# axiom-crypto/halo2-lib

Hardware: AMD Instinct MI355X
Metric: create_proof constraints/sec (k=19 ECDSA configuration, halo2-ecc/configs/secp256k1/bench_ecdsa.config:1); MSM G1-adds/sec in `msm_2_20` (higher is better)
Workload: dtype u32 (254-bit Montgomery integers as 8x32 / 9x29-bit limbs); 1 GPU; BASELINE configs[3]: h2hip_plonk_create_proof, k=19 secp256k1-ECDSA shape (bench_ecdsa.config:1: 1 advice + 1 lookup + 1 constants column, lookup_bits 18), synthetic circuit-like witness resident in HBM; 1 step = 1 proof, bytes back on the host; constraints_per_proof=524280, msm_count=12, msm_size=524288, extended_k=21, degree=5, proof_bytes=960

## Files before the change

### halo2-lib_amd/csrc/internal.h

```cpp
#pragma once
#include <hip/hip_runtime.h>
#include <stdint.h>
#include <stdio.h>
#include <string.h>
#include <functional>
#include <map>
#include <string>
#include <vector>

#include "../../include/h2hip.h"
#include "ec.cuh"
#include "ec29.cuh"

namespace h2 {

void set_error(const char *fmt, ...);

#define H2_HIPCHK(expr)                                                                              \
    do {                                                                                             \
        hipError_t e__ = (expr);                                                                     \
        if (e__ != hipSuccess) {                                                                     \
            h2::set_error("%s:%d: %s -> %s", __FILE__, __LINE__, #expr, hipGetErrorString(e__));     \
            return H2HIP_ERR_HIP;                                                                    \
        }                                                                                            \
    } while (0)

#define H2_CHK(expr)                      \
    do {                                  \
        int r__ = (expr);                 \
        if (r__ != H2HIP_OK) return r__;  \
    } while (0)

#define H2_REQUIRE(cond, msg)                                        \
    do {                                                             \
        if (!(cond)) {                                               \
            h2::set_error("%s: invalid argument: %s", __func__, msg); \
            return H2HIP_ERR_INVALID;                                \
        }                                                            \
    } while (0)

struct DevBuf {
    void *p = nullptr;
    size_t cap = 0;
};

struct TwiddleSet {
    uint32_t log_n = 0, lo_bits = 0;
    Fr omega;
    void *t1 = nullptr;
    void *t2 = nullptr;
    void *direct[4] = {nullptr, nullptr, nullptr, nullptr};
    uint32_t direct_log_s[4] = {0, 0, 0, 0};
};

struct KernelStat {
    double total_ms = 0;
    uint64_t launches = 0;
    std::vector<std::pair<float, float>> spans;
};

}

struct h2hip_ctx {
    int device = 0;
    hipStream_t stream = nullptr;
    bool own_stream = false;
    int num_cus = 256;
    enum { WS_NTT = 0, WS_DIGITS, WS_COUNTS, WS_OFFSETS, WS_CURSOR, WS_SKEY, WS_SVAL, WS_BUCKETS, WS_PKEY0, WS_PVAL0, WS_PKEY1,
           WS_PVAL1, WS_SEG, WS_WIN, WS_OUT, WS_SCAN, WS_TMP0, WS_TMP1, WS_TMP2, WS_STAGE, WS_POSEIDON, WS_FBTABLE, WS_BATCH, WS_LK0, WS_LK1, WS_LK2, WS_LK3, WS_LK4, WS_LK5, WS_VANISH, WS_BATCH_BUCKETS, WS_COUNT };
    h2::DevBuf ws[WS_COUNT];
    std::vector<h2::TwiddleSet> twiddles;
    int msm_window_bits = 0;
    int msm_chunk = 0;
    int msm_seg = 4;
    int ntt_tile_bits = 10;
    int ntt_min_col_bits = 2;
    int ntt_full_table = 1;
    int ntt_tile_kernel = 1;
    int ntt_debug_skip = 0;
    int msm_quad_tails = 1;
    int msm_sort_threads = 1024;
    int msm_scatter_split = 0;
    int msm_scatter_full_lds = 0;
    bool is_lane = false;
    int msm_chunk_lone = -1;
    int msm_hist_split = 0;
    int msm_sort_groups = 0;
    int msm_hist_packed = 1;
    uint32_t pos_t = 0, pos_rf = 0, pos_rp = 0;
    bool profiling = false;
    std::string prof_filter;
    std::map<std::string, h2::KernelStat> stats;
    struct PendingLaunch {
        std::string name;
        hipEvent_t begin, end;
        bool ended;
    };
    std::vector<PendingLaunch> pending;
    std::vector<hipEvent_t> event_pool;
    hipEvent_t prof_ref = nullptr;
    bool own_prof_ref = false;
    h2hip_ctx *lane[4] = {nullptr, nullptr, nullptr, nullptr};
    hipEvent_t lane_ev[4] = {nullptr, nullptr, nullptr, nullptr};
    char *job_ring = nullptr;
    size_t job_ring_off = 0;
    std::function<int()> msm_mid_hook;
    size_t msm_mid_after = 0;
    std::function<int(size_t)> msm_col_hook;
    hipEvent_t fork_ev3 = nullptr;
    int plonk_lazy_upload = 1;
    hipEvent_t fork_ev2 = nullptr;
    std::function<int(hipEvent_t ev)> msm_tail_hook;
    hipEvent_t tail_ev = nullptr;
    int msm_lanes = 0;
    int plonk_tail_overlap = 1;
    int quotient_29 = 1;
    int plonk_permute_in_commit = 1;
    int clean_on_lane = 1;
    int kate_29 = 1;
    int kate_coeffs_per_lane = 0;
    int plonk_merge_products = 1;
    int plonk_shard_side = 1;
    int plonk_route_rows = 1;
    int plonk_early_intt = 1;
    int plonk_gate_before_join = 0;
    int msm_stagger_sorts = -1;
    hipEvent_t sorted_ev = nullptr;
    bool sorted_arm = false;
    int plonk_side_on_lanes = 1;
#ifdef H2_HIPEMU
    int plonk_warm_keygen = 0;
#else
    int plonk_warm_keygen = 1;
#endif
    int fr_invert_run = 0;
    int lookup_big_tile_bits = 19;
    int msm_quad_seg_max = 32768;
    int msm_defer_reduce = 1;
    int msm_fuse_cols = 0;
    hipStream_t clean_stream = nullptr;
    hipEvent_t clean_ev = nullptr, clean_ev1 = nullptr, used_ev = nullptr;
    void *clean_ptr[2] = {nullptr, nullptr};
    size_t clean_bytes[2] = {0, 0};
    hipEvent_t fork_ev = nullptr;
    hipEvent_t timer_ev[2] = {nullptr, nullptr};
    int msm_table_split = 1;
    int host_poll = 1;
    char *poll_host = nullptr;
    char *poll_dev = nullptr;
    unsigned long long poll_seq = 0;
    bool msm_lds_attr_set = false, lookup_lds_attr_set = false, ntt_lds_attr_set = false;
};

namespace h2 {
inline bool knob_pow2(int v) { return v > 0 && (v & (v - 1)) == 0; }
}
#define H2_INHERITED true
#define H2_PARENT_ONLY(why) false
#define H2_KNOB_TABLE(K)                                                                                                                          \
    K(msm_window_bits, H2_INHERITED, v == 0 || (v >= 4 && v <= 16), "0 (auto) or 4..16")                                                         \
    K(msm_chunk, H2_INHERITED, v == 0 || (v >= 2 && v <= 4096), "0 (auto) or 2..4096")                                                          \
    K(msm_chunk_lone, H2_INHERITED, v >= -1 && v <= 4096, "-1 (auto), 0 (the batch rule) or 1..4096")                                          \
    K(msm_seg, H2_INHERITED, h2::knob_pow2(v) && v <= 1024, "a power of two <= 1024")                                                          \
    K(msm_quad_tails, H2_INHERITED, v == 0 || v == 1, "0 or 1")                                                                                 \
    K(msm_quad_seg_max, H2_INHERITED, v >= 0, ">= 0")                                                                                           \
    K(msm_sort_threads, H2_INHERITED, v == 256 || v == 512 || v == 1024, "256, 512 or 1024")                                                   \
    K(msm_sort_groups, H2_INHERITED, v >= 0 && v <= 1024, "0 (auto) or 1..1024")                                                               \
    K(msm_hist_split, H2_INHERITED, v == 0 || (h2::knob_pow2(v) && v <= 64), "0 or a power of two <= 64")                                      \
    K(msm_hist_packed, H2_INHERITED, v == 0 || v == 1, "0 or 1")                                                                                \
    K(msm_scatter_split, H2_INHERITED, v == 0 || (h2::knob_pow2(v) && v <= 64), "0 (auto) or a power of two <= 64")                            \
    K(msm_scatter_full_lds, H2_INHERITED, v == 0 || v == 1, "0 or 1")                                                                           \
    K(msm_table_split, H2_INHERITED, v == 0 || v == 1, "0 or 1")                                                                                \
    K(msm_lanes, H2_PARENT_ONLY("read only by the batch driver, on the caller's context"), v >= 0 && v <= 4, "0 (auto) or 1..4")              \
    K(msm_stagger_sorts, H2_PARENT_ONLY("read only by the batch driver, on the caller's context"), v >= -1 && v <= 1, "-1 (auto), 0 or 1")     \
    K(msm_fuse_cols, H2_PARENT_ONLY("read only by the batch driver, on the caller's context"), v >= 0 && v <= (int)h2::MSM_MAX_COLS,           \
      "0 (auto) or 1..32")                                                                                                                        \
    K(msm_defer_reduce, H2_PARENT_ONLY("read only by the batch driver, on the caller's context"), v == 0 || v == 1, "0 or 1")                  \
    K(clean_on_lane, H2_PARENT_ONLY("read only by the batch driver, on the caller's context"), v == 0 || v == 1, "0 or 1")                     \
    K(ntt_tile_bits, H2_INHERITED, v >= 4 && v <= 10, "4..10")                                                                                  \
    K(ntt_min_col_bits, H2_INHERITED, v >= 0 && v <= 5, "0..5")                                                                                 \
    K(ntt_full_table, H2_INHERITED, v == 0 || v == 1, "0 or 1")                                                                                 \
    K(ntt_tile_kernel, H2_INHERITED, v == 0 || v == 1, "0 or 1")                                                                                \
    K(ntt_debug_skip, H2_INHERITED, v >= 0 && v <= 2, "0, 1 or 2")                                                                              \
    K(quotient_29, H2_INHERITED, v == 0 || v == 1, "0 or 1")                                                                                    \
    K(kate_29, H2_INHERITED, v == 0 || v == 1, "0 or 1")                                                                                        \
    K(kate_coeffs_per_lane, H2_INHERITED, v == 0 || v == 1 || v == 2 || v == 4 || v == 8, "0 (by length), 1, 2, 4 or 8")                       \
    K(fr_invert_run, H2_INHERITED, v >= 0 && v <= 1024, "0 (auto) or 1..1024")                                                                 \
    K(lookup_big_tile_bits, H2_INHERITED, v >= 12 && v <= 28, "12..28")                                                                         \
    K(host_poll, H2_INHERITED, v == 0 || v == 1, "0 or 1")                                                                                      \
    K(plonk_warm_keygen, H2_PARENT_ONLY("read only by h2hip_plonk_keygen"), v == 0 || v == 1, "0 or 1")                                       \
    K(plonk_tail_overlap, H2_PARENT_ONLY("read only by create_proof, on the caller's context"), v == 0 || v == 1, "0 or 1")                    \
    K(plonk_side_on_lanes, H2_PARENT_ONLY("read only by create_proof, on the caller's context"), v == 0 || v == 1, "0 or 1")                   \
    K(plonk_permute_in_commit, H2_PARENT_ONLY("read only by create_proof, on the caller's context"), v == 0 || v == 1, "0 or 1")               \
    K(plonk_merge_products, H2_PARENT_ONLY("read only by create_proof, on the caller's context"), v == 0 || v == 1, "0 or 1")                  \
    K(plonk_shard_side, H2_PARENT_ONLY("read only by create_proof, on the caller's context"), v >= 0 && v <= 2, "0, 1 or 2 (forced)")          \
    K(plonk_route_rows, H2_PARENT_ONLY("read only by create_proof, on the caller's context"), v == 0 || v == 1, "0 or 1")                      \
    K(plonk_lazy_upload, H2_PARENT_ONLY("read only by create_proof, on the caller's context"), v == 0 || v == 1, "0 or 1")                     \
    K(plonk_early_intt, H2_PARENT_ONLY("read only by create_proof, on the caller's context"), v == 0 || v == 1, "0 or 1")                      \
    K(plonk_gate_before_join, H2_PARENT_ONLY("read only by create_proof, on the caller's context"), v == 0 || v == 1, "0 or 1")

namespace h2 {
inline void inherit_knobs(h2hip_ctx *c, const h2hip_ctx *p) {
#define H2_KNOB_INHERIT(name, inherit, legal, domain) \
    if (inherit) c->name = p->name;
    H2_KNOB_TABLE(H2_KNOB_INHERIT)
#undef H2_KNOB_INHERIT
    c->profiling = p->profiling;
    c->prof_filter = p->prof_filter;
    c->prof_ref = p->prof_ref;
}
struct DeviceGuard {
    int prev = -1;
    bool switched = false;
    explicit DeviceGuard(const h2hip_ctx *c) {
        if (c && hipGetDevice(&prev) == hipSuccess && prev != c->device) switched = hipSetDevice(c->device) == hipSuccess;
    }
    ~DeviceGuard() {
        if (switched) hipSetDevice(prev);
    }
    DeviceGuard(const DeviceGuard &) = delete;
    DeviceGuard &operator=(const DeviceGuard &) = delete;
};
}
#define H2_DEVICE_GUARD(ctx) h2::DeviceGuard device_guard__(ctx)

struct h2hip_bases {
    h2::G1Affine *pts = nullptr;
    h2::G1Affine *pts29 = nullptr;
    bool split = false;
    size_t n = 0;
    uint32_t window_bits = 0;
    uint32_t tables = 1;
};

namespace h2 {
struct alignas(128) TableEntry29 {
    uint32_t x[9], y[9];
    uint32_t pad[14];
};
static_assert(sizeof(TableEntry29) == 128, "one entry per 128-byte line");
int ws_reserve(h2hip_ctx *ctx, int slot, size_t bytes, void **out);

void prof_begin(h2hip_ctx *ctx, const char *name);
void prof_end(h2hip_ctx *ctx);
bool prof_launch_events(h2hip_ctx *ctx, const char *name, hipEvent_t *start, hipEvent_t *stop);

int ntt_run(h2hip_ctx *ctx, Fr *a, uint32_t log_n, const Fr &omega, const Fr *in_override, uint64_t in_len, const Fr *in_scale3,
            const Fr *out_scale3);
int ntt_run_batch(h2hip_ctx *ctx, Fr *const *a, const Fr *const *in_override, size_t ncols, uint32_t log_n, const Fr &omega, uint64_t in_len,
                  const Fr *in_scale3, const Fr *out_scale3);
constexpr uint32_t LK_COMPRESS_MAX_EXPRS = 49, LK_COMPRESS_MAX_WIDTH = 5;
int lookup_compress_batch_dev(h2hip_ctx *ctx, const Fr *const *cols, Fr *const *out, uint32_t count, uint32_t width, size_t rows, const Fr &theta);
int fr_scatter_rows(h2hip_ctx *ctx, Fr *const *dst, size_t count, const Fr *src, size_t src_stride, size_t len);
int upload_jobs(h2hip_ctx *ctx, void *dst_dev, const void *src_host, size_t bytes);
int exclusive_scan_u32_segments(h2hip_ctx *ctx, const uint32_t *in, uint32_t *out, uint32_t n, uint32_t segments, size_t in_stride,
                                size_t out_stride);
int exclusive_scan_u32(h2hip_ctx *ctx, const uint32_t *in, uint32_t *out, uint32_t n);
int batch_normalize_jac(h2hip_ctx *ctx, const G1Jac *tmp, G1Affine *out, uint32_t n);
uint32_t pick_window(size_t n, bool precomp = false);
int msm_prepare_bases(h2hip_ctx *ctx, h2hip_bases *bases, bool precompute);
int msm_run(h2hip_ctx *ctx, const h2hip_bases *bases, const Fr *scalars_dev, size_t n, XYZZ *out_dev);
constexpr uint32_t MSM_MAX_COLS = 32;
int msm_run_cols(h2hip_ctx *ctx, const h2hip_bases *bases, const Fr *const *scalars_dev, uint32_t ncols, size_t n, XYZZ *out_dev,
                 XYZZ29 *ext_buckets, bool ext_buckets_zeroed = false);
bool buckets_prezeroed(h2hip_ctx *ctx, int which, const void *buf, size_t bytes);
int buckets_clean_after_use(h2hip_ctx *ctx, int which, void *buf, size_t bytes, hipStream_t on = nullptr);
int sync_stream(h2hip_ctx *ctx);
int sync_results(h2hip_ctx *ctx, void *dst_host, const void *src_dev, size_t bytes);
void prof_fold_child(h2hip_ctx *parent, h2hip_ctx *child);
int rng_chacha_fill_dev(h2hip_ctx *ctx, Fr *out_dev, size_t n, const uint8_t seed[32], int rounds, uint64_t first_block, hipStream_t stream);
int comm_reserve_allgather_dev(h2hip_comm *comm, size_t bytes);
int comm_reserve_alltoall_dev(h2hip_comm *c, size_t bytes);
int plonk_phased_layout(const h2hip_phased_circuit_params &pp, h2hip_plonk_shape *shape, std::vector<std::vector<int>> *phase_cols,
                        uint32_t challenges[H2HIP_MAX_PHASE], bool *phased, h2hip_base_circuit_params *bp);
int msm_reduce_cols(h2hip_ctx *ctx, const h2hip_bases *bases, uint32_t window_bits, const XYZZ29 *buckets, uint32_t ncols, XYZZ *out_dev);
uint32_t lookup_padded_keys(uint32_t u);
int lookup_sort_keys_dev(h2hip_ctx *ctx, void *keys, uint32_t N);
struct WitnessCheckJob {
    uint32_t u = 0;
    std::vector<const Fr *> cols;
    std::vector<uint32_t> gate_adv, gate_q;
    std::vector<uint32_t> gate_report;
    std::vector<uint32_t> lk_in, lk_q;
    const void *table_sorted = nullptr;
    uint32_t dyn_width = 0;
    std::vector<uint32_t> dyn_in, dyn_tab;
    uint32_t num_lookups = 0;
    std::vector<uint32_t> perm_col;
    const uint16_t *sigma_c = nullptr;
    const uint32_t *sigma_r = nullptr;
};
constexpr uint32_t WC_NONE = 0xFFFFFFFFu;
int witness_check_run(h2hip_ctx *ctx, const WitnessCheckJob &job, h2hip_witness_failure *failures_out, size_t max_failures, size_t *num_failures);
}
```

### halo2-lib_amd/csrc/msm.hip

```cpp
#include "internal.h"
#ifndef H2_HIPEMU
#include <hip/hip_ext.h>
#endif
#include "ec29.cuh"
#include "quad29.cuh"

namespace h2 {

#ifdef H2_HIPEMU
#define H2_TAIL_PRIORITY() ((void)0)
#define H2_SORT_PRIORITY() ((void)0)
#else
#define H2_TAIL_PRIORITY() __builtin_amdgcn_s_setprio(3)
#define H2_SORT_PRIORITY() __builtin_amdgcn_s_setprio(2)
#endif


constexpr uint32_t KEY_INVALID = 0xFFFFFFFFu;
constexpr uint32_t MAX_LDS_BUCKETS = 1u << 15;

struct DigitCols {
    const Fr *scalars[MSM_MAX_COLS];
};
typedef uint16_t digit_t;
// ... 345 lines not shown
        const uint32_t oh = __shfl(head ? 1u : 0u, (int)(lane >= d ? lane - d : lane));
        if (need) {
            xyzz29_add(acc, other);
            head = oh != 0;
        }
    }
    const uint32_t src1 = lane ? lane - 1 : 0;
    const uint32_t prev_head = __shfl(head ? 1u : 0u, (int)src1);
    const bool pull = multi && l_open && lane > 0;
    XYZZ29 lval = XYZZ29::identity();
    if (multi) lval = lsave[threadIdx.x];
    if (multi && !l_open) {
        buckets[hk] = lval;
        lval = XYZZ29::identity();
    }
    if ((__any(pull ? 1 : 0) != 0)) {
        const XYZZ29 prev = xyzz29_shfl(acc, src1);
        if (pull) xyzz29_add(lval, prev);
    }
    bool left_mine = false, right_mine = false;
    uint32_t pkey = KEY_INVALID;
    XYZZ29 pv = XYZZ29::identity();
    if (multi && l_open) {
        if (lane > 0 && prev_head) {
            if (!lval.is_identity()) buckets[hk] = lval;
        } else {
            left_mine = true;
            pkey = hk;
            pv = lval;
        }
    }
    const uint32_t next_valid = __shfl(valid ? 1u : 0u, (int)(lane < 63 ? lane + 1 : lane));
    const bool last_valid = valid && (lane == 63 || !next_valid);
    if (valid) {
        if (r_open && last_valid) {
            right_mine = true;
        } else if (!r_open) {
            if (head) {
                if (!acc.is_identity()) buckets[cur] = acc;
            } else {
                left_mine = true;
                pkey = cur;
                pv = acc;
            }
        }
    }
    const bool any_left = (__any(left_mine ? 1 : 0) != 0);
    if (left_mine) {
        out_keys[2 * (size_t)wave] = pkey;
        out_vals[2 * (size_t)wave] = pv;
    } else if (lane == 0 && !any_left) {
        out_keys[2 * (size_t)wave] = first_key;
        if (first_key != KEY_INVALID) out_vals[2 * (size_t)wave] = XYZZ29::identity();
    }
    const bool any_valid = (__any(valid ? 1 : 0) != 0);
    if (right_mine) {
        out_keys[2 * (size_t)wave + 1] = cur;
        out_vals[2 * (size_t)wave + 1] = acc;
    } else if (last_valid) {
        out_keys[2 * (size_t)wave + 1] = cur;
        out_vals[2 * (size_t)wave + 1] = XYZZ29::identity();
    } else if (lane == 0 && !any_valid) {
        out_keys[2 * (size_t)wave + 1] = KEY_INVALID;
    }
}

template <bool SPLIT>
__global__ __launch_bounds__(256, 3) void msm_accum_kernel(const uint32_t *__restrict__ sval, const G1Affine *__restrict__ bases,
                                                          const uint32_t *__restrict__ offsets, uint32_t nkeys, uint32_t K,
                                                          XYZZ29 *__restrict__ buckets, uint32_t *__restrict__ out_keys,
                                                          XYZZ29 *__restrict__ out_vals, uint32_t nthreads) {
    msm_accum_body<SPLIT>(sval, bases, offsets, nkeys, K, buckets, out_keys, out_vals, nthreads);
}

__global__ __launch_bounds__(256) void msm_merge_kernel(const uint32_t *__restrict__ kin, const XYZZ29 *__restrict__ vin, uint32_t len,
                                                        XYZZ29 *__restrict__ buckets, uint32_t *__restrict__ kout,
                                                        XYZZ29 *__restrict__ vout, uint32_t final_level) {
    H2_TAIL_PRIORITY();
    __shared__ XYZZ29 sv[256];
    __shared__ uint32_t sk[256];
    const uint32_t tid = threadIdx.x, blk = blockIdx.x;
    const uint32_t i = blk * 256 + tid;
    const uint32_t key = i < len ? kin[i] : KEY_INVALID;
    XYZZ29 val = XYZZ29::identity();
    if (key != KEY_INVALID) val = vin[i];
    sk[tid] = key;
    sv[tid] = val;
    __syncthreads();
    for (uint32_t d = 1; d < 256; d <<= 1) {
        const bool m = tid >= d && key != KEY_INVALID && sk[tid - d] == key;
        XYZZ29 other = XYZZ29::identity();
        if (m) other = sv[tid - d];
        if (!__syncthreads_or(m ? 1 : 0)) break;
        if (m) {
            xyzz29_add(val, other);
            sv[tid] = val;
        }
        __syncthreads();
    }
    const uint32_t first_key = sk[0], last_key = sk[255];
    if (!final_level && tid == 0) {
        kout[2 * (size_t)blk] = first_key;
        vout[2 * (size_t)blk] = XYZZ29::identity();
        kout[2 * (size_t)blk + 1] = last_key;
        if (last_key != KEY_INVALID) vout[2 * (size_t)blk + 1] = XYZZ29::identity();
    }
    __syncthreads();
    if (key == KEY_INVALID) return;
    const bool in_block_end = (tid == 255) || (sk[tid + 1] != key);
    if (!in_block_end) return;
    bool left_closed = true, right_closed = true;
    if (!final_level) {
        if (key == first_key && blk > 0) left_closed = kin[blk * 256 - 1] != key;
        if (tid == 255) right_closed = (i + 1 >= len) || (kin[i + 1] != key);
    }
    if (left_closed && right_closed) {
        if (!val.is_identity()) buckets[key] = val;
    } else if (key == first_key) {
        vout[2 * (size_t)blk] = val;
    } else {
        vout[2 * (size_t)blk + 1] = val;
    }
}

__device__ __forceinline__ XYZZ29 xyzz_small_mul(const XYZZ29 &p, uint32_t k) {
    XYZZ29 r = XYZZ29::identity();
    for (int bit = 31 - __clz(k | 1u); bit >= 0; --bit) {
        r = xyzz29_double(r);
        if ((k >> bit) & 1u) xyzz29_add(r, p);
    }
    return r;
}
__global__ __launch_bounds__(64) void msm_presum_kernel(const XYZZ29 *__restrict__ in, XYZZ29 *__restrict__ out, uint32_t B, uint32_t rows,
                                                        uint32_t group) {
    H2_TAIL_PRIORITY();
    uint32_t t = blockIdx.x * blockDim.x + threadIdx.x;
    uint32_t groups = (rows + group - 1) / group;
    if (t >= B * groups) return;
    in += (size_t)blockIdx.y * rows * B;
    out += (size_t)blockIdx.y * groups * B;
    uint32_t gi = t / B, b = t - gi * B;
    uint32_t w0 = gi * group, w1 = w0 + group < rows ? w0 + group : rows;
    XYZZ29 acc = in[(size_t)w0 * B + b];
    for (uint32_t w = w0 + 1; w < w1; ++w) xyzz29_add(acc, in[(size_t)w * B + b]);
    out[(size_t)gi * B + b] = acc;
}
__global__ __launch_bounds__(64) void msm_seg_kernel(const XYZZ29 *__restrict__ buckets, XYZZ29 *__restrict__ seg_out, uint32_t B, uint32_t L,
                                                     uint32_t nseg_total) {
    H2_TAIL_PRIORITY();
    uint32_t g = blockIdx.x * blockDim.x + threadIdx.x;
    if (g >= nseg_total) return;
    uint32_t per = B / L, w = g / per, lo = (g - w * per) * L;
    const XYZZ29 *bw = buckets + (size_t)w * B;
    XYZZ29 run = XYZZ29::identity(), acc = XYZZ29::identity();
    for (int b = (int)(lo + L) - 1; b >= (int)lo; --b) {
        xyzz29_add(run, bw[b]);
        xyzz29_add(acc, run);
    }
    if (lo) xyzz29_add(acc, xyzz_small_mul(run, lo));
    seg_out[g] = acc;
}
__global__ __launch_bounds__(1024) void msm_winsum_kernel(const XYZZ29 *__restrict__ seg, XYZZ29 *__restrict__ win_out, uint32_t per) {
    H2_TAIL_PRIORITY();
    __shared__ XYZZ29 sh[1024];
    uint32_t tid = threadIdx.x, w = blockIdx.x;
    XYZZ29 acc = XYZZ29::identity();
    for (uint32_t i = tid; i < per; i += 1024) xyzz29_add(acc, seg[(size_t)w * per + i]);
    sh[tid] = acc;
    __syncthreads();
    for (uint32_t d = 512; d >= 1; d >>= 1) {
        if (tid < d) {
            XYZZ29 a = sh[tid];
            xyzz29_add(a, sh[tid + d]);
            sh[tid] = a;
        }
        __syncthreads();
    }
    if (tid == 0) win_out[w] = sh[0];
}
__global__ __launch_bounds__(64) void msm_fold_kernel(const XYZZ29 *__restrict__ win, uint32_t Wr, uint32_t c, XYZZ *__restrict__ out) {
    H2_TAIL_PRIORITY();
    __shared__ XYZZ29 sh[64];
    uint32_t tid = threadIdx.x;
    XYZZ29 p = XYZZ29::identity();
    if (tid < Wr) {
        p = win[tid];
        for (uint32_t i = 0; i < c * tid; ++i) p = xyzz29_double(p);
    }
    sh[tid] = p;
    __syncthreads();
    for (uint32_t d = 32; d >= 1; d >>= 1) {
        if (tid < d) {
            XYZZ29 a = sh[tid];
            xyzz29_add(a, sh[tid + d]);
            sh[tid] = a;
        }
        __syncthreads();
    }
    if (tid == 0) out[0] = xyzz29_to_sat(sh[0]);
}


__global__ __launch_bounds__(256) void msm_seg_quad_kernel(const XYZZ29 *__restrict__ buckets, XYZZ29 *__restrict__ seg_out, uint32_t B, uint32_t L,
                                                           uint32_t nseg_total, uint32_t lo_bits, uint32_t tree) {
    H2_TAIL_PRIORITY();
    __shared__ XYZZ29 sh[64];
    const uint32_t lane = threadIdx.x & 63u, q = lane & 3u, qi = threadIdx.x >> 2;
    uint32_t g = blockIdx.x * 64 + qi;
    const bool live = g < nseg_total;
    if (!live) g = nseg_total - 1;
    uint32_t per = B / L, w = g / per, lo = (g - w * per) * L;
    const XYZZ29 *bw = buckets + (size_t)w * B;
    Fq29 run = Fq29::zero(), acc = Fq29::zero();
    for (int b = (int)(lo + L) - 1; b >= (int)lo; --b) {
        run = quad_xyzz_add(run, quad_load(bw + b, q), lane);
        acc = quad_xyzz_add(acc, run, lane);
    }
    acc = quad_xyzz_add(acc, quad_xyzz_small_mul(run, lo, lo_bits, lane), lane);
    if (!tree) {
        if (live) quad_store(seg_out + g, q, acc);
        return;
    }
    if (!live) acc = Fq29::zero();
    quad_store(&sh[qi], q, acc);
    __syncthreads();
    for (uint32_t d = 32; d >= 1; d >>= 1) {
        Fq29 other = quad_load(&sh[(qi + d) & 63u], q);
        Fq29 sum = quad_xyzz_add(acc, other, lane);
        __syncthreads();
        if (qi < d) {
            acc = sum;
            quad_store(&sh[qi], q, acc);
        }
        __syncthreads();
    }
    if (qi == 0) quad_store(seg_out + blockIdx.x, q, acc);
}
template <int THREADS>
__global__ __launch_bounds__(THREADS) void msm_winsum_quad_kernel(const XYZZ29 *__restrict__ seg, XYZZ29 *__restrict__ win_out, uint32_t per) {
    H2_TAIL_PRIORITY();
    constexpr uint32_t NQ = THREADS / 4;
    __shared__ XYZZ29 sh[NQ];
    const uint32_t lane = threadIdx.x & 63u, q = lane & 3u, qi = threadIdx.x >> 2, w = blockIdx.x;
    Fq29 acc = Fq29::zero();
    const uint32_t rounds = (per + NQ - 1) / NQ;
    for (uint32_t r = 0; r < rounds; ++r) {
        uint32_t i = qi + NQ * r;
        Fq29 v = i < per ? quad_load(seg + (size_t)w * per + i, q) : Fq29::zero();
        acc = rounds == 1 ? v : quad_xyzz_add(acc, v, lane);
    }
    quad_store(&sh[qi], q, acc);
    __syncthreads();
    uint32_t d0 = NQ / 2;
    while (d0 > 1 && d0 >= per) d0 >>= 1;
    if (per <= 1) d0 = 0;
    for (uint32_t d = d0; d >= 1; d >>= 1) {
        Fq29 other = qi + d < NQ ? quad_load(&sh[qi + d], q) : Fq29::zero();
        Fq29 sum = quad_xyzz_add(acc, other, lane);
        __syncthreads();
        if (qi < d) {
            acc = sum;
            quad_store(&sh[qi], q, acc);
        }
        __syncthreads();
    }
    if (qi == 0) quad_store(win_out + w, q, acc);
}

__global__ __launch_bounds__(256) void msm_fold_quad_kernel(const XYZZ29 *__restrict__ win, uint32_t Wr, uint32_t c, XYZZ *__restrict__ out) {
    H2_TAIL_PRIORITY();
    __shared__ XYZZ29 sh[64];
    const uint32_t lane = threadIdx.x & 63u, q = lane & 3u, qi = threadIdx.x >> 2;
    Fq29 p = qi < Wr ? quad_load(win + qi, q) : Fq29::zero();
    const uint32_t max_dbl = c * (Wr - 1);
    for (uint32_t i = 0; i < max_dbl; ++i) {
        Fq29 d = quad_xyzz_double(p, lane);
        p = f29_select(i < c * qi && qi < Wr, d, p);
    }
    quad_store(&sh[qi], q, p);
    __syncthreads();
    for (uint32_t d = 32; d >= 1; d >>= 1) {
        Fq29 other = quad_load(&sh[(qi + d) & 63u], q);
        Fq29 sum = quad_xyzz_add(p, other, lane);
        __syncthreads();
        if (qi < d) {
            p = sum;
            quad_store(&sh[qi], q, p);
        }
        __syncthreads();
    }
    if (qi == 0) {
        const bool id = quad_is_identity(p, lane);
        Fq v = id ? Fq::zero() : f29_to_sat(p);
        reinterpret_cast<Fq *>(out)[q] = v;
    }
}

__global__ __launch_bounds__(64) void msm_cols_out_kernel(const XYZZ29 *__restrict__ win, uint32_t ncols, XYZZ *__restrict__ out) {
    H2_TAIL_PRIORITY();
    uint32_t col = blockIdx.x * blockDim.x + threadIdx.x;
    if (col < ncols) out[col] = xyzz29_to_sat(win[col]);
}

int msm_reduce_cols(h2hip_ctx *ctx, const h2hip_bases *bases, uint32_t c, const XYZZ29 *buckets, uint32_t ncols, XYZZ *out) {
    hipStream_t st = ctx->stream;
    const bool precomp = bases->tables > 1;
    H2_REQUIRE(ncols >= 1 && ncols <= 64 && (ncols == 1 || precomp), "1..64 bucket sets (several need precomputed bases)");
    const uint32_t Wcol = (255 + c - 1) / c, B = 1u << (c - 1);
    uint32_t L = (uint32_t)ctx->msm_seg;
    if (L > B) L = B;
    const uint32_t Wr = precomp ? ncols : Wcol;
    const uint32_t nseg = Wr * (B / L);
    XYZZ29 *seg, *win, *presum = nullptr;
    H2_CHK(ws_reserve(ctx, h2hip_ctx::WS_SEG, sizeof(XYZZ29) * nseg, (void **)&seg));
    H2_CHK(ws_reserve(ctx, h2hip_ctx::WS_WIN, sizeof(XYZZ29) * 64, (void **)&win));
    const uint32_t rows = precomp ? Wcol : 1;
    const uint32_t pre_rows = (rows + 3) / 4;
    if (precomp && rows > 1) H2_CHK(ws_reserve(ctx, h2hip_ctx::WS_TMP0, sizeof(XYZZ29) * B * (size_t)ncols * (pre_rows + 1), (void **)&presum));
    const XYZZ29 *red_in = buckets;
    if (precomp && rows > 1) {
        prof_begin(ctx, "msm_presum_kernel");
        if (rows <= 4) {
            hipLaunchKernelGGL(msm_presum_kernel, dim3((B + 63) / 64, ncols), dim3(64), 0, st, buckets, presum, B, rows, rows);
        } else {
            XYZZ29 *stage1 = presum + (size_t)ncols * B;
            hipLaunchKernelGGL(msm_presum_kernel, dim3((B * pre_rows + 63) / 64, ncols), dim3(64), 0, st, buckets, stage1, B, rows, 4u);
            hipLaunchKernelGGL(msm_presum_kernel, dim3((B + 63) / 64, ncols), dim3(64), 0, st, (const XYZZ29 *)stage1, presum, B, pre_rows, pre_rows);
        }
        prof_end(ctx);
        red_in = presum;
    }
    const bool quad_reduce = ctx->msm_quad_tails && nseg <= (uint32_t)ctx->msm_quad_seg_max;
    if (quad_reduce) {
        uint32_t lo_bits = 0;
        while ((1u << lo_bits) < B) ++lo_bits;
        const uint32_t per = B / L;
        const uint32_t tree = (per % 64 == 0) ? 1u : 0u;
        prof_begin(ctx, "msm_seg_kernel");
        hipLaunchKernelGGL(msm_seg_quad_kernel, dim3((nseg + 63) / 64), dim3(256), 0, st, red_in, seg, B, L, nseg, lo_bits, tree);
        prof_end(ctx);
        prof_begin(ctx, "msm_winsum_kernel");
        const uint32_t wper = tree ? per / 64 : per;
        if (wper <= 128)
            hipLaunchKernelGGL(msm_winsum_quad_kernel<256>, dim3(Wr), dim3(256), 0, st, (const XYZZ29 *)seg, win, wper);
        else
            hipLaunchKernelGGL(msm_winsum_quad_kernel<1024>, dim3(Wr), dim3(1024), 0, st, (const XYZZ29 *)seg, win, wper);
        prof_end(ctx);
    } else {
        prof_begin(ctx, "msm_seg_kernel");
        hipLaunchKernelGGL(msm_seg_kernel, dim3((nseg + 63) / 64), dim3(64), 0, st, red_in, seg, B, L, nseg);
        prof_end(ctx);
        prof_begin(ctx, "msm_winsum_kernel");
        hipLaunchKernelGGL(msm_winsum_kernel, dim3(Wr), dim3(1024), 0, st, (const XYZZ29 *)seg, win, B / L);
        prof_end(ctx);
    }
    prof_begin(ctx, "msm_fold_kernel");
    if (precomp) {
        hipLaunchKernelGGL(msm_cols_out_kernel, dim3(1), dim3(64), 0, st, (const XYZZ29 *)win, ncols, out);
    } else if (ctx->msm_quad_tails) {
        hipLaunchKernelGGL(msm_fold_quad_kernel, dim3(1), dim3(256), 0, st, (const XYZZ29 *)win, Wr, c, out);
    } else {
        hipLaunchKernelGGL(msm_fold_kernel, dim3(1), dim3(64), 0, st, (const XYZZ29 *)win, Wr, c, out);
    }
    prof_end(ctx);
    H2_HIPCHK(hipGetLastError());
    return H2HIP_OK;
}

bool buckets_prezeroed(h2hip_ctx *ctx, int which, const void *buf, size_t bytes) {
    const bool ok = ctx->clean_ev && ctx->clean_ptr[which] == buf && ctx->clean_bytes[which] >= bytes;
    if (ok) ctx->clean_bytes[which] = 0;
    return ok;
}
int buckets_clean_after_use(h2hip_ctx *ctx, int which, void *buf, size_t bytes, hipStream_t on) {
    if (!ctx->clean_stream) {
        H2_HIPCHK(hipStreamCreateWithFlags(&ctx->clean_stream, hipStreamNonBlocking));
        H2_HIPCHK(hipEventCreateWithFlags(&ctx->clean_ev, hipEventDisableTiming));
        H2_HIPCHK(hipEventCreateWithFlags(&ctx->clean_ev1, hipEventDisableTiming));
        H2_HIPCHK(hipEventCreateWithFlags(&ctx->used_ev, hipEventDisableTiming));
    }
    const hipStream_t cs = on ? on : ctx->clean_stream;
    H2_HIPCHK(hipEventRecord(ctx->used_ev, ctx->stream));
    H2_HIPCHK(hipStreamWaitEvent(cs, ctx->used_ev, 0));
    H2_HIPCHK(hipMemsetAsync(buf, 0, bytes, cs));
    H2_HIPCHK(hipEventRecord(which ? ctx->clean_ev1 : ctx->clean_ev, cs));
    ctx->clean_ptr[which] = buf;
    ctx->clean_bytes[which] = bytes;
    return H2HIP_OK;
}

int msm_run_cols(h2hip_ctx *ctx, const h2hip_bases *bases, const Fr *const *scalars, uint32_t ncols, size_t n, XYZZ *out, XYZZ29 *ext_buckets,
                 bool ext_buckets_zeroed) {
    H2_REQUIRE(ncols >= 1 && ncols <= MSM_MAX_COLS, "1..32 columns per fused MSM");
    H2_REQUIRE(n <= bases->n, "more scalars than resident bases");
    H2_REQUIRE(bases->pts29 != nullptr || bases->n == 0, "bases are not prepared");
    H2_REQUIRE(n < (1u << 27), "n too large for 32-bit entry indices");
    hipStream_t st = ctx->stream;
    if (n == 0) {
        H2_REQUIRE(!ext_buckets, "empty MSM in a deferred-reduction batch");
        H2_HIPCHK(hipMemsetAsync(out, 0, sizeof(XYZZ) * ncols, st));
        return H2HIP_OK;
    }
    const bool precomp = bases->tables > 1;
    H2_REQUIRE(ncols == 1 || precomp, "a fused multi-column MSM needs precomputed bases");
    const uint32_t c = precomp ? bases->window_bits : (ctx->msm_window_bits ? (uint32_t)ctx->msm_window_bits : pick_window(n));
    H2_REQUIRE(c >= 2 && c <= 16, "window bits must be 2..16 (a window's bucket histogram lives in LDS)");
    const uint32_t Wcol = (255 + c - 1) / c;
    H2_REQUIRE(Wcol <= 64, "too many windows");
    H2_REQUIRE(!precomp || bases->tables >= Wcol, "precomputed table has too few windows");
    const uint32_t W = Wcol * ncols;
    const G1Affine *table = (const G1Affine *)bases->pts29;
    const uint32_t B = 1u << (c - 1);
    const uint32_t nkeys = W * B;
    const uint64_t emax = (uint64_t)n * W;
    H2_REQUIRE(emax < 0xFFFFFFF0ull, "n*W overflows 32 bits");
    uint32_t K1 = (uint32_t)ctx->msm_chunk;
    if (K1 == 0) {
        uint64_t k = emax / 262144;
        K1 = k < 8 ? 8u : k > 64 ? 64u : (uint32_t)k;
        const bool lone = !ctx->is_lane && ctx->msm_chunk_lone != 0;
        if (lone) {
            if (ctx->msm_chunk_lone > 0) K1 = (uint32_t)ctx->msm_chunk_lone;
        } else if (emax >= 25000000ull) K1 = 64;
        else if (emax >= 12000000ull) K1 = 32;
        else if (emax >= 4000000ull) K1 = 24;
    }
    const uint32_t sort_groups = ctx->msm_sort_groups > 0 ? (uint32_t)ctx->msm_sort_groups : 32u;
    uint32_t chunk = (uint32_t)((n + sort_groups - 1) / sort_groups);
    if (chunk < 4096) chunk = 4096;
    const uint32_t chunk_cap = ctx->msm_hist_packed ? 65535u : 65536u;
    if (chunk > chunk_cap) chunk = chunk_cap;
    const uint32_t G = (uint32_t)((n + chunk - 1) / chunk);

    digit_t *digits;
    uint32_t *bhist, *counts, *offsets, *sval, *pkey[2];
    XYZZ29 *buckets, *pval[2];
    H2_CHK(ws_reserve(ctx, h2hip_ctx::WS_DIGITS, sizeof(digit_t) * emax, (void **)&digits));
    H2_CHK(ws_reserve(ctx, h2hip_ctx::WS_CURSOR, sizeof(uint32_t) * (size_t)W * G * B, (void **)&bhist));
    H2_CHK(ws_reserve(ctx, h2hip_ctx::WS_COUNTS, sizeof(uint32_t) * ((size_t)nkeys + 1), (void **)&counts));
    H2_CHK(ws_reserve(ctx, h2hip_ctx::WS_OFFSETS, sizeof(uint32_t) * ((size_t)nkeys + 2), (void **)&offsets));
    H2_CHK(ws_reserve(ctx, h2hip_ctx::WS_SVAL, sizeof(uint32_t) * (emax + 4), (void **)&sval));
    if (ext_buckets) buckets = ext_buckets;
    else H2_CHK(ws_reserve(ctx, h2hip_ctx::WS_BUCKETS, sizeof(XYZZ29) * nkeys, (void **)&buckets));
    const uint32_t T1 = (uint32_t)((emax + K1 - 1) / K1);
    const uint32_t accum_blocks = (T1 + 255) / 256;
    const uint32_t len1 = 8 * accum_blocks, blocks1 = (len1 + 255) / 256;
    H2_CHK(ws_reserve(ctx, h2hip_ctx::WS_PKEY0, sizeof(uint32_t) * (size_t)len1, (void **)&pkey[0]));
    H2_CHK(ws_reserve(ctx, h2hip_ctx::WS_PVAL0, sizeof(XYZZ29) * (size_t)len1, (void **)&pval[0]));
    H2_CHK(ws_reserve(ctx, h2hip_ctx::WS_PKEY1, sizeof(uint32_t) * 2 * (size_t)blocks1, (void **)&pkey[1]));
    H2_CHK(ws_reserve(ctx, h2hip_ctx::WS_PVAL1, sizeof(XYZZ29) * 2 * (size_t)blocks1, (void **)&pval[1]));

    if (ext_buckets) {
        if (!ext_buckets_zeroed) H2_HIPCHK(hipMemsetAsync(buckets, 0, sizeof(XYZZ29) * nkeys, st));
    } else if (buckets_prezeroed(ctx, 0, buckets, sizeof(XYZZ29) * nkeys)) {
        H2_HIPCHK(hipStreamWaitEvent(st, ctx->clean_ev, 0));
    } else {
        H2_HIPCHK(hipMemsetAsync(buckets, 0, sizeof(XYZZ29) * nkeys, st));
    }
    DigitCols dcols;
    for (uint32_t col = 0; col < MSM_MAX_COLS; ++col) {
        H2_REQUIRE(col >= ncols || scalars[col], "NULL scalar column");
        dcols.scalars[col] = col < ncols ? scalars[col] : nullptr;
    }
    prof_begin(ctx, "msm_digits_kernel");
    hipLaunchKernelGGL(msm_digits_kernel, dim3((uint32_t)((n + 255) / 256), ncols), dim3(256), 0, st, dcols, (uint32_t)n, c, Wcol, digits, counts + nkeys,
                       offsets + nkeys + 1);
    prof_end(ctx);
    const uint32_t sort_threads = (uint32_t)ctx->msm_sort_threads;
    if (!ctx->msm_lds_attr_set) {
        H2_HIPCHK(hipFuncSetAttribute((const void *)msm_hist_kernel<false>, hipFuncAttributeMaxDynamicSharedMemorySize, (int)(sizeof(uint32_t) * MAX_LDS_BUCKETS)));
        H2_HIPCHK(hipFuncSetAttribute((const void *)msm_hist_kernel<true>, hipFuncAttributeMaxDynamicSharedMemorySize, (int)(sizeof(uint32_t) * MAX_LDS_BUCKETS)));
        H2_HIPCHK(hipFuncSetAttribute((const void *)msm_scatter_kernel, hipFuncAttributeMaxDynamicSharedMemorySize, (int)(sizeof(uint32_t) * MAX_LDS_BUCKETS)));
        ctx->msm_lds_attr_set = true;
    }
    prof_begin(ctx, "msm_hist_kernel");
    const bool hist_packed = ctx->msm_hist_packed != 0 && chunk < 65536u && B >= 2;
    uint32_t HS = ctx->msm_hist_split > 0 ? (uint32_t)ctx->msm_hist_split : 1u;
    if (HS > B) HS = B;
    const uint32_t hist_grid = sort_grid_size(W * HS, G);
    if (hist_packed)
        hipLaunchKernelGGL(msm_hist_kernel<true>, dim3(hist_grid), dim3(sort_threads), sizeof(uint32_t) * ((B / HS + 1) / 2), st, (const digit_t *)digits, (uint32_t)n, W, B, G, chunk, HS, bhist);
    else
        hipLaunchKernelGGL(msm_hist_kernel<false>, dim3(hist_grid), dim3(sort_threads), sizeof(uint32_t) * (B / HS), st, (const digit_t *)digits, (uint32_t)n, W, B, G, chunk, HS, bhist);
    prof_end(ctx);
    prof_begin(ctx, "msm_hist_scan_kernel");
    hipLaunchKernelGGL(msm_hist_scan_kernel, dim3((nkeys + 255) / 256), dim3(256), 0, st, bhist, W, B, G, counts);
    prof_end(ctx);
    H2_HIPCHK(hipGetLastError());
    H2_CHK(exclusive_scan_u32(ctx, counts, offsets, nkeys + 1));
    prof_begin(ctx, "msm_scatter_kernel");
    uint32_t S = (uint32_t)ctx->msm_scatter_split;
    if (S == 0) {
        S = 1;
        while (S < 4 && S * 2 <= B && ((uint64_t)n * 4) / S > (2u << 20)) S *= 2;
    }
    if (S > B) S = B;
    const uint32_t scatter_grid = sort_grid_size(W * S, G);
    hipLaunchKernelGGL(msm_scatter_kernel, dim3(scatter_grid), dim3(sort_threads), ctx->msm_scatter_full_lds ? sizeof(uint32_t) * MAX_LDS_BUCKETS : sizeof(uint32_t) * (B / S), st,
                       (const digit_t *)digits, (uint32_t)n, W, B, G, chunk, S, precomp ? (uint32_t)bases->n : 0u, Wcol, (const uint32_t *)offsets,
                       (const uint32_t *)bhist, sval);
    prof_end(ctx);
    H2_HIPCHK(hipGetLastError());
    if (ctx->sorted_arm) {
        ctx->sorted_arm = false;
        H2_HIPCHK(hipEventRecord(ctx->sorted_ev, st));
    }

    {
        hipEvent_t ev_a = nullptr, ev_b = nullptr;
#ifndef H2_HIPEMU
        if (prof_launch_events(ctx, "msm_accum_kernel", &ev_a, &ev_b)) {
            if (bases->split)
                hipExtLaunchKernelGGL(msm_accum_kernel<true>, dim3(accum_blocks), dim3(256), 0, st, ev_a, ev_b, 0, (const uint32_t *)sval, table,
                                      (const uint32_t *)offsets, nkeys, K1, buckets, pkey[0], pval[0], T1);
            else
                hipExtLaunchKernelGGL(msm_accum_kernel<false>, dim3(accum_blocks), dim3(256), 0, st, ev_a, ev_b, 0, (const uint32_t *)sval, table,
                                      (const uint32_t *)offsets, nkeys, K1, buckets, pkey[0], pval[0], T1);
        } else
#endif
        {
            prof_begin(ctx, "msm_accum_kernel");
            if (bases->split)
                hipLaunchKernelGGL(msm_accum_kernel<true>, dim3(accum_blocks), dim3(256), 0, st, (const uint32_t *)sval, table, (const uint32_t *)offsets, nkeys, K1,
                                   buckets, pkey[0], pval[0], T1);
            else
                hipLaunchKernelGGL(msm_accum_kernel<false>, dim3(accum_blocks), dim3(256), 0, st, (const uint32_t *)sval, table, (const uint32_t *)offsets, nkeys, K1,
                                   buckets, pkey[0], pval[0], T1);
            prof_end(ctx);
        }
        (void)ev_a;
        (void)ev_b;
    }
    H2_HIPCHK(hipGetLastError());
    uint32_t len = len1;
    int src = 0;
    for (;;) {
        const uint32_t blocks = (len + 255) / 256;
        const uint32_t final_level = blocks == 1 ? 1u : 0u;
        prof_begin(ctx, "msm_merge_kernel");
        hipLaunchKernelGGL(msm_merge_kernel, dim3(blocks), dim3(256), 0, st, (const uint32_t *)pkey[src], (const XYZZ29 *)pval[src], len, buckets,
                           pkey[src ^ 1], pval[src ^ 1], final_level);
        prof_end(ctx);
        H2_HIPCHK(hipGetLastError());
        if (final_level) break;
        len = 2 * blocks;
        src ^= 1;
    }

    if (ext_buckets) return H2HIP_OK;
    H2_CHK(msm_reduce_cols(ctx, bases, c, buckets, ncols, out));
    return buckets_clean_after_use(ctx, 0, buckets, sizeof(XYZZ29) * nkeys);
}

int msm_run(h2hip_ctx *ctx, const h2hip_bases *bases, const Fr *scalars, size_t n, XYZZ *out) {
    return msm_run_cols(ctx, bases, &scalars, 1, n, out, nullptr, false);
}

}
```

Before: 39.43 million constraints/s.

## Reduce precomputed MSM bucket sets with split-bit line sums instead of running sums

```diff
diff --git a/halo2-lib_amd/csrc/internal.h b/halo2-lib_amd/csrc/internal.h
--- a/halo2-lib_amd/csrc/internal.h
+++ b/halo2-lib_amd/csrc/internal.h
@@ -161,7 +161,7 @@
     K(msm_window_bits, H2_INHERITED, v == 0 || (v >= 4 && v <= 16), "0 (auto) or 4..16")                                                         \
     K(msm_chunk, H2_INHERITED, v == 0 || (v >= 2 && v <= 4096), "0 (auto) or 2..4096")                                                          \
     K(msm_chunk_lone, H2_INHERITED, v >= -1 && v <= 4096, "-1 (auto), 0 (the batch rule) or 1..4096")                                          \
-    K(msm_seg, H2_INHERITED, h2::knob_pow2(v) && v <= 1024, "a power of two <= 1024")                                                          \
+    K(msm_seg, H2_INHERITED, v == -1 || (h2::knob_pow2(v) && v <= 1024), "-1 or a power of two <= 1024")                                      \
     K(msm_quad_tails, H2_INHERITED, v == 0 || v == 1, "0 or 1")                                                                                 \
     K(msm_quad_seg_max, H2_INHERITED, v >= 0, ">= 0")                                                                                           \
     K(msm_sort_threads, H2_INHERITED, v == 256 || v == 512 || v == 1024, "256, 512 or 1024")                                                   \
diff --git a/halo2-lib_amd/csrc/msm.hip b/halo2-lib_amd/csrc/msm.hip
--- a/halo2-lib_amd/csrc/msm.hip
+++ b/halo2-lib_amd/csrc/msm.hip
@@ -671,17 +671,120 @@
     if (col < ncols) out[col] = xyzz29_to_sat(win[col]);
 }
 
+
+template <uint32_t NQ, class At>
+__device__ __forceinline__ Fq29 quad_block_sum(XYZZ29 *sh, uint32_t count, uint32_t qi, uint32_t q, uint32_t lane, At at) {
+    Fq29 acc = Fq29::zero();
+    const uint32_t rounds = (count + NQ - 1) / NQ;
+    for (uint32_t r = 0; r < rounds; ++r) {
+        const uint32_t i = qi + NQ * r;
+        const Fq29 v = i < count ? quad_load(at(i), q) : Fq29::zero();
+        acc = r == 0 ? v : quad_xyzz_add(acc, v, lane);
+    }
+    const uint32_t active = count < NQ ? count : NQ;
+    if (active <= 1) return acc;
+    uint32_t d0 = 1;
+    while (2 * d0 < active) d0 <<= 1;
+    quad_store(&sh[qi], q, acc);
+    __syncthreads();
+    for (uint32_t d = d0; d >= 1; d >>= 1) {
+        const Fq29 other = qi + d < NQ ? quad_load(&sh[qi + d], q) : Fq29::zero();
+        const Fq29 sum = quad_xyzz_add(acc, other, lane);
+        __syncthreads();
+        if (qi < d) {
+            acc = sum;
+            quad_store(&sh[qi], q, acc);
+        }
+        __syncthreads();
+    }
+    return acc;
+}
+
+__global__ __launch_bounds__(256) void msm_split_lines_kernel(const XYZZ29 *__restrict__ sets, XYZZ29 *__restrict__ lines, uint32_t *__restrict__ arrived,
+                                                              uint32_t lo_bits, uint32_t hi_bits) {
+    H2_TAIL_PRIORITY();
+    __shared__ XYZZ29 sh[64];
+    const uint32_t lane = threadIdx.x & 63u, q = lane & 3u, qi = threadIdx.x >> 2, x = blockIdx.x, col = blockIdx.y;
+    const uint32_t NL = 1u << lo_bits, NH = 1u << hi_bits;
+    if (x == 0 && threadIdx.x == 0) arrived[col] = 0;
+    const XYZZ29 *s = sets + ((size_t)col << (lo_bits + hi_bits));
+    const bool row = x < NH;
+    const XYZZ29 *first = row ? s + ((size_t)x << lo_bits) : s + (x - NH);
+    const uint32_t stride = row ? 1u : NL;
+    const Fq29 acc = quad_block_sum<64>(sh, row ? NL : NH, qi, q, lane, [&](uint32_t i) { return first + (size_t)i * stride; });
+    if (qi == 0) quad_store(lines + (size_t)col * (NH + NL) + x, q, acc);
+}
+
+__device__ __forceinline__ uint32_t split_arrive(uint32_t *counter) {
+#ifdef H2_HIPEMU
+    __threadfence();
+    return atomicAdd(counter, 1u);
+#else
+    __builtin_amdgcn_fence(__ATOMIC_RELEASE, "agent");
+    asm volatile("s_waitcnt vmcnt(0)" ::: "memory");
+    return __hip_atomic_fetch_add(counter, 1u, __ATOMIC_RELAXED, __HIP_MEMORY_SCOPE_AGENT);
+#endif
+}
+__device__ __forceinline__ void split_acquire() {
+#ifdef H2_HIPEMU
+    __threadfence();
+#else
+    __builtin_amdgcn_fence(__ATOMIC_ACQUIRE, "agent");
+    asm volatile("s_waitcnt vmcnt(0)" ::: "memory");
+#endif
+}
+
+__global__ __launch_bounds__(128) void msm_split_bits_kernel(const XYZZ29 *__restrict__ lines, XYZZ29 *__restrict__ parts, uint32_t *__restrict__ arrived,
+                                                             uint32_t lo_bits, uint32_t hi_bits, XYZZ *__restrict__ out) {
+    H2_TAIL_PRIORITY();
+    __shared__ XYZZ29 sh[32];
+    __shared__ uint32_t last;
+    const uint32_t lane = threadIdx.x & 63u, q = lane & 3u, qi = threadIdx.x >> 2, s = blockIdx.x, col = blockIdx.y;
+    const uint32_t NL = 1u << lo_bits, NH = 1u << hi_bits, nsum = lo_bits + hi_bits + 1;
+    const XYZZ29 *ln = lines + (size_t)col * (NH + NL);
+    const bool lo_side = s <= lo_bits;
+    const XYZZ29 *src = lo_side ? ln + NH : ln;
+    const uint32_t bit = s == 0 ? 0u : lo_side ? s - 1 : s - 1 - lo_bits, setv = s == 0 ? 0u : 1u;
+    const uint32_t below = (1u << bit) - 1u;
+    Fq29 acc = quad_block_sum<32>(sh, (lo_side ? NL : NH) / 2, qi, q, lane,
+                                  [&](uint32_t i) { return src + (((i & ~below) << 1) | (setv << bit) | (i & below)); });
+    const uint32_t dbl = s == 0 ? 0u : s == 1 ? 1u : s - 1;
+    for (uint32_t i = 0; i < dbl; ++i) acc = quad_xyzz_double(acc, lane);
+    XYZZ29 *pc = parts + (size_t)col * nsum;
+    if (qi == 0) quad_store(pc + s, q, acc);
+#ifndef H2_HIPEMU
+    asm volatile("s_waitcnt vmcnt(0)" ::: "memory");
+#endif
+    __syncthreads();
+    if (threadIdx.x == 0) {
+        last = split_arrive(arrived + col) == nsum - 1 ? 1u : 0u;
+        if (last) split_acquire();
+    }
+    __syncthreads();
+    if (!last) return;
+    acc = quad_block_sum<32>(sh, nsum, qi, q, lane, [&](uint32_t i) { return pc + i; });
+    if (qi == 0) {
+        const bool id = quad_is_identity(acc, lane);
+        const Fq v = id ? Fq::zero() : f29_to_sat(acc);
+        reinterpret_cast<Fq *>(out + col)[q] = v;
+    }
+}
+
 int msm_reduce_cols(h2hip_ctx *ctx, const h2hip_bases *bases, uint32_t c, const XYZZ29 *buckets, uint32_t ncols, XYZZ *out) {
     hipStream_t st = ctx->stream;
     const bool precomp = bases->tables > 1;
     H2_REQUIRE(ncols >= 1 && ncols <= 64 && (ncols == 1 || precomp), "1..64 bucket sets (several need precomputed bases)");
     const uint32_t Wcol = (255 + c - 1) / c, B = 1u << (c - 1);
-    uint32_t L = (uint32_t)ctx->msm_seg;
+    uint32_t L = ctx->msm_seg > 0 ? (uint32_t)ctx->msm_seg : 4u;
     if (L > B) L = B;
     const uint32_t Wr = precomp ? ncols : Wcol;
     const uint32_t nseg = Wr * (B / L);
+    const bool quad_reduce = ctx->msm_quad_tails && nseg <= (uint32_t)ctx->msm_quad_seg_max;
+    const bool split = precomp && quad_reduce && c >= 3 && ctx->msm_seg > 0;
+    const uint32_t lo_bits = (c - 1) / 2, hi_bits = (c - 1) - lo_bits, nlines = (1u << lo_bits) + (1u << hi_bits);
+    const size_t nsplit = (size_t)ncols * (nlines + c);
     XYZZ29 *seg, *win, *presum = nullptr;
-    H2_CHK(ws_reserve(ctx, h2hip_ctx::WS_SEG, sizeof(XYZZ29) * nseg, (void **)&seg));
+    H2_CHK(ws_reserve(ctx, h2hip_ctx::WS_SEG, sizeof(XYZZ29) * (split && nsplit > nseg ? nsplit : nseg), (void **)&seg));
     H2_CHK(ws_reserve(ctx, h2hip_ctx::WS_WIN, sizeof(XYZZ29) * 64, (void **)&win));
     const uint32_t rows = precomp ? Wcol : 1;
     const uint32_t pre_rows = (rows + 3) / 4;
@@ -699,7 +802,18 @@
         prof_end(ctx);
         red_in = presum;
     }
-    const bool quad_reduce = ctx->msm_quad_tails && nseg <= (uint32_t)ctx->msm_quad_seg_max;
+    if (split) {
+        XYZZ29 *lines = seg, *parts = seg + (size_t)ncols * nlines;
+        uint32_t *arrived = (uint32_t *)win;
+        prof_begin(ctx, "msm_seg_kernel");
+        hipLaunchKernelGGL(msm_split_lines_kernel, dim3(nlines, ncols), dim3(256), 0, st, red_in, lines, arrived, lo_bits, hi_bits);
+        prof_end(ctx);
+        prof_begin(ctx, "msm_winsum_kernel");
+        hipLaunchKernelGGL(msm_split_bits_kernel, dim3(c, ncols), dim3(128), 0, st, (const XYZZ29 *)lines, parts, arrived, lo_bits, hi_bits, out);
+        prof_end(ctx);
+        H2_HIPCHK(hipGetLastError());
+        return H2HIP_OK;
+    }
     if (quad_reduce) {
         uint32_t lo_bits = 0;
         while ((1u << lo_bits) < B) ++lo_bits;
```

Result: faster. 40.15 million constraints/s (median of 4 runs) (+1.8%).
